# helixml/helix

Measured on AMD Instinct MI355X. Metric: tokens/sec, higher is better.
Workload: dtype bf16; 1 GPU; model=llama3-8b, global_batch=512, seq_len=512, parallelism=dp1, kv_cache_dtype=bf16

## Files before the change

### helix_amd/engine/engine.py

```python
from __future__ import annotations

import time
import zlib
from dataclasses import dataclass, field
from enum import Enum
from typing import Callable, Dict, List, Optional

import numpy as np
import torch

from helix_amd import ops
from helix_amd.engine.kv_cache import KVCache, chain_hash
from helix_amd.engine.sampling_params import SamplingParams
from helix_amd.models.llama import (DecodeMeta, LlamaConfig, LlamaForCausalLM,
                                    PrefillMeta, PRESETS)

_SEED_MIX = 0x9E3779B97F4A7C15


class SeqStatus(Enum):
    WAITING = "waiting"
    RUNNING = "running"
    FINISHED = "finished"
    CANCELLED = "cancelled"


@dataclass
class Sequence:
    seq_id: str
    prompt_ids: List[int]
    params: SamplingParams
    output_ids: List[int] = field(default_factory=list)
    status: SeqStatus = SeqStatus.WAITING
    block_table: List[int] = field(default_factory=list)
    row: int = -1
    cached_prefix: int = 0
    block_hashes: List[bytes] = field(default_factory=list)
    arrival_time: float = field(default_factory=time.monotonic)
    first_token_time: Optional[float] = None
    finish_reason: Optional[str] = None
    logprobs: List[dict] = field(default_factory=list)
    pen_init: bool = False
    json_mask: object = None
    on_token: Optional[Callable] = None
    lora: Optional[str] = None

    @property
    def total_len(self) -> int:
        return len(self.prompt_ids) + len(self.output_ids)


@dataclass
class EngineConfig:
    model: str = "llama3-8b"
    block_size: int = 16
    max_num_seqs: int = 64
    max_model_len: int = 8192
    max_prefill_tokens: int = 8192
    kv_cache_blocks: Optional[int] = None
    gpu_memory_utilization: float = 0.90
    eos_token_id: int = 2
    seed: int = 0
    enforce_eager: bool = False
    enable_prefix_caching: bool = True
    quantization: Optional[str] = None
    kv_cache_dtype: str = "bf16"
    max_loras: int = 0
    max_lora_rank: int = 16


class LLMEngine:
    def __init__(self, cfg: EngineConfig, device: str = "cuda",
                 model: Optional[LlamaForCausalLM] = None,
                 tp_size: int = 1, tp_rank: int = 0,
                 tp_group=None):
        self.cfg = cfg
        self.device = torch.device(device)
        self.model_cfg: LlamaConfig = PRESETS[cfg.model]
        self.tp_size = tp_size
        self.tp_rank = tp_rank
        self.tp_group = tp_group
        if model is None:
            dtype = torch.bfloat16
            model = LlamaForCausalLM(self.model_cfg, tp_size, tp_rank)
            model = model.to(dtype).to(self.device)
            model.init_random(cfg.seed)
        if cfg.quantization == "fp8":
            from helix_amd.models.quant import quantize_model_fp8
            quantize_model_fp8(model)
        elif cfg.quantization in ("q4_0", "q8_0", "q4_k", "q6_k"):
            from helix_amd.models.quant import has_wq, quantize_model_wq
            if not has_wq(model):
                quantize_model_wq(model, cfg.quantization)
        from helix_amd.models.quant import attach_wq_scratch
        attach_wq_scratch(model)
        self.model = model
        self.lora = None
        if cfg.max_loras > 0:
            if tp_size > 1:
                raise ValueError(
                    "max_loras > 0 is not supported with tp_size > 1 "
                    "(tensor-parallel-sharded adapters are not implemented)")
            from helix_amd.models.lora import LoRAManager
            self.lora = LoRAManager(model, cfg.max_loras, cfg.max_lora_rank)

        nkv = self.model_cfg.num_kv_heads // tp_size
        num_blocks = cfg.kv_cache_blocks
        if num_blocks is None:
            num_blocks = self._auto_kv_blocks(nkv)
        kv_dtype = torch.uint8 if cfg.kv_cache_dtype == "fp8" \
            else torch.bfloat16
        self.kv = KVCache(self.model_cfg.num_layers, nkv,
                          self.model_cfg.head_dim, cfg.block_size, num_blocks,
                          self.device, dtype=kv_dtype)
        self.waiting: List[Sequence] = []
        self.running: List[Sequence] = []
        self.seqs: Dict[str, Sequence] = {}
        self.steps = 0
        if self.device.type == "cuda":
            self.decode_ws = ops.decode_workspace(
                cfg.max_num_seqs, self.model_cfg.num_heads // tp_size,
                self.model_cfg.head_dim, cfg.max_model_len, self.device)
        else:
            self.decode_ws = None
        self._pen_counts: Optional[torch.Tensor] = None
        self._pen_seen: Optional[torch.Tensor] = None
        if self.device.type == "cuda":
            R = cfg.max_num_seqs
            self._samp_hf = torch.empty(5, R, dtype=torch.float32,
                                        pin_memory=True)
            self._samp_hs = torch.empty(R, dtype=torch.int64,
                                        pin_memory=True)
            self._samp_hi = torch.empty(2, R, dtype=torch.int32,
                                        pin_memory=True)
            self._samp_df = torch.empty(5, R, dtype=torch.float32,
                                        device=self.device)
            self._samp_ds = torch.empty(R, dtype=torch.int64,
                                        device=self.device)
            self._samp_di = torch.empty(2, R, dtype=torch.int32,
                                        device=self.device)
        mb = cfg.max_model_len // cfg.block_size + 2
        self._bt_np = np.zeros((cfg.max_num_seqs, mb), dtype=np.int32)
        self._free_rows = list(range(cfg.max_num_seqs - 1, -1, -1))
        self._ids_np = np.zeros(cfg.max_num_seqs, dtype=np.int64)
        self._pos_np = np.zeros(cfg.max_num_seqs, dtype=np.int64)
        self._slots_np = np.zeros(cfg.max_num_seqs, dtype=np.int64)
        self._lens_np = np.zeros(cfg.max_num_seqs, dtype=np.int32)
        self._rows_np = np.zeros(cfg.max_num_seqs, dtype=np.intp)
        self._lora_np = np.full(cfg.max_num_seqs, -1, dtype=np.int32)
        self.graph_runner = None
        if self.device.type == "cuda" and not cfg.enforce_eager:
            from helix_amd.engine.graph_runner import CUDAGraphRunner
            self.graph_runner = CUDAGraphRunner(
                self.model, self.kv.caches, self.decode_ws,
                cfg.max_model_len, cfg.block_size, cfg.max_num_seqs,
                self.device, lora=self.lora is not None)

    def _auto_kv_blocks(self, nkv: int) -> int:
        if self.device.type != "cuda":
            return 512
        free, total = torch.cuda.mem_get_info(self.device)
        budget = int(total * self.cfg.gpu_memory_utilization
                     - (total - free))
        budget = max(budget, 1 << 28)
        n = KVCache.blocks_for_bytes(budget, self.model_cfg.num_layers, nkv,
                                     self.model_cfg.head_dim,
                                     self.cfg.block_size)
        cap = (self.cfg.max_num_seqs *
               (self.cfg.max_model_len // self.cfg.block_size + 1))
        return max(1, min(n, cap))

    def add_request(self, seq_id: str, prompt_ids: List[int],
                    params: SamplingParams,
                    on_token: Optional[Callable] = None,
                    lora: Optional[str] = None) -> Sequence:
        if len(prompt_ids) >= self.cfg.max_model_len:
            raise ValueError(
                f"prompt length {len(prompt_ids)} >= max_model_len "
                f"{self.cfg.max_model_len}")
        if lora is not None:
            if self.lora is None:
                raise ValueError(
                    f"LoRA adapter {lora!r} requested but the engine was "
                    "built with max_loras=0")
            if lora not in self.lora.adapters:
                raise ValueError(f"unknown LoRA adapter {lora!r}")
        seq = Sequence(seq_id=seq_id, prompt_ids=list(prompt_ids),
                       params=params, on_token=on_token, lora=lora)
        self.seqs[seq_id] = seq
        self.waiting.append(seq)
        return seq

    def _lora_in_use(self, name: str) -> bool:
        return any(s.lora == name for s in self.waiting + self.running)

    def add_lora(self, name: str, path: str):
        if self.lora is None:
            raise ValueError("engine was built with max_loras=0")
        if self._lora_in_use(name):
            raise ValueError(
                f"LoRA adapter {name!r} is referenced by queued or running "
                "sequences; cannot reload it")
        self.lora.add(name, path)

    def remove_lora(self, name: str):
        if self.lora is None or name not in self.lora.adapters:
            raise ValueError(f"unknown LoRA adapter {name!r}")
        if self._lora_in_use(name):
            raise ValueError(
                f"LoRA adapter {name!r} is referenced by queued or running "
                "sequences; cannot remove it")
        self.lora.remove(name)

    def list_loras(self) -> List[str]:
        return self.lora.names() if self.lora is not None else []

    def _pinned_loras(self, batch: List[Sequence]) -> set:
        pinned = {s.lora for s in self.running if s.lora}
        pinned.update(s.lora for s in batch if s.lora)
        pinned.update(s.lora for s in self.waiting
                      if s.lora and s.block_table)
        return pinned

    def _lora_slots(self, lora_names) -> Optional[List[int]]:
        if self.lora is None or not any(lora_names):
            return None
        out = []
        for n in lora_names:
            s = self.lora.slot_of(n)
            if n is not None and s < 0:
                raise RuntimeError(f"LoRA adapter {n!r} is not resident")
            out.append(s)
        return out

    def cancel(self, seq_id: str):
        seq = self.seqs.get(seq_id)
        if seq is None:
            return
        if seq.status == SeqStatus.WAITING:
            self.waiting.remove(seq)
            if seq.block_table:
                self.kv.allocator.free(seq.block_table)
                seq.block_table = []
                self._release_row(seq)
        elif seq.status == SeqStatus.RUNNING:
            self.running.remove(seq)
            self.kv.allocator.free(seq.block_table)
            seq.block_table = []
            self._release_row(seq)
        seq.status = SeqStatus.CANCELLED
        seq.finish_reason = "cancelled"

    @property
    def has_work(self) -> bool:
        return bool(self.waiting or self.running)

    def num_free_blocks(self) -> int:
        return self.kv.allocator.free_count

    def step(self) -> List[tuple]:
        prefill_batch = self._schedule_prefill()
        if prefill_batch:
            out = self._run_prefill(prefill_batch)
        elif self.running:
            out = self._run_decode()
        else:
            return []
        self.steps += 1
        events = []
        for seq, tok in out:
            finished = self._append_token(seq, tok)
            events.append((seq, tok, finished))
            if seq.on_token is not None:
                seq.on_token(seq, tok, finished)
        return events

    def _schedule_prefill(self) -> List[Sequence]:
        batch: List[Sequence] = []
        tokens = 0
        bs = self.cfg.block_size
        alloc = self.kv.allocator
        self._chunk_target: Dict[str, int] = {}
        while self.waiting and len(self.running) + len(batch) < self.cfg.max_num_seqs:
            seq = self.waiting[0]
            L = len(seq.prompt_ids)
            first = not seq.block_table
            if seq.lora is not None and self.lora.acquire(
                    seq.lora, self._pinned_loras(batch)) < 0:
                break
            matched: List[int] = []
            if first:
                if self.cfg.enable_prefix_caching:
                    if not seq.block_hashes:
                        h = b"" if seq.lora is None \
                            else self.lora.hash_seed(seq.lora)
                        for i in range(L // bs):
                            h = chain_hash(h,
                                           seq.prompt_ids[i * bs:(i + 1) * bs])
                            seq.block_hashes.append(h)
                    for h in seq.block_hashes:
                        b = alloc.lookup_hash(h)
                        if b is None:
                            break
                        matched.append(b)
                    while matched and len(matched) * bs > L - 1:
                        matched.pop()
                P = len(matched) * bs
            else:
                P = seq.cached_prefix
            budget = self.cfg.max_prefill_tokens - tokens
            if budget <= 0:
                break
            T = min(L, P + budget)
            if T <= P:
                break
            if batch and T < L:
                break
            nblocks = (T + bs - 1) // bs
            new_blocks = nblocks - max(len(seq.block_table), len(matched))
            head = 1 if T == L else 0
            if not alloc.can_allocate(new_blocks + head):
                break
            if first:
                seq.block_table = [alloc.share(b) for b in matched] + \
                    alloc.allocate(new_blocks)
            else:
                seq.block_table.extend(alloc.allocate(new_blocks))
            self._assign_row(seq)
            seq.cached_prefix = P
            self._chunk_target[seq.seq_id] = T
            if T == L:
                batch.append(self.waiting.pop(0))
            else:
                batch.append(seq)
            tokens += T - P
            if T < L:
                break
        return batch

    def _slot(self, seq: Sequence, pos: int) -> int:
        bs = self.cfg.block_size
        return seq.block_table[pos // bs] * bs + pos % bs

    def _assign_row(self, seq: Sequence):
        if seq.row < 0:
            seq.row = self._free_rows.pop()
        n = len(seq.block_table)
        self._bt_np[seq.row, :n] = seq.block_table
        self._bt_np[seq.row, n:] = 0

    def _release_row(self, seq: Sequence):
        if seq.row >= 0:
            self._free_rows.append(seq.row)
            seq.row = -1
        seq.pen_init = False

    def _run_prefill(self, batch: List[Sequence]):
        bs = self.cfg.block_size
        input_ids, positions, slots, cu_q, cu_k = [], [], [], [0], [0]
        gather_blk, gather_off = [], []
        row_slots = self._lora_slots([s.lora for s in batch])
        tok_slots: List[int] = []
        targets = getattr(self, "_chunk_target", {})
        any_cached = any(s.cached_prefix for s in batch)
        for seq in batch:
            L = targets.get(seq.seq_id, len(seq.prompt_ids))
            P = seq.cached_prefix
            input_ids.extend(seq.prompt_ids[P:L])
            positions.extend(range(P, L))
            slots.extend(self._slot(seq, p) for p in range(P, L))
            cu_q.append(cu_q[-1] + L - P)
            cu_k.append(cu_k[-1] + L)
            if row_slots is not None:
                tok_slots.extend([row_slots[len(cu_q) - 2]] * (L - P))
            if any_cached:
                for p in range(L):
                    gather_blk.append(seq.block_table[p // bs])
                    gather_off.append(p % bs)
        dev = self.device
        meta = PrefillMeta(
            cu_seqlens=torch.tensor(cu_q, dtype=torch.int32, device=dev),
            max_seqlen=max(targets.get(s.seq_id, len(s.prompt_ids))
                           - s.cached_prefix for s in batch),
            slot_mapping=torch.tensor(slots, dtype=torch.int64, device=dev),
            positions=torch.tensor(positions, dtype=torch.int64, device=dev),
            cu_seqlens_k=(torch.tensor(cu_k, dtype=torch.int32, device=dev)
                          if any_cached else None),
            gather_blk=(torch.tensor(gather_blk, dtype=torch.int64,
                                     device=dev) if any_cached else None),
            gather_off=(torch.tensor(gather_off, dtype=torch.int64,
                                     device=dev) if any_cached else None),
            lora_slots=(torch.tensor(tok_slots, dtype=torch.int32,
                                     device=dev)
                        if row_slots is not None else None))
        ids = torch.tensor(input_ids, dtype=torch.int64, device=dev)
        hidden = self.model(ids, self.kv.caches, meta)
        if self.cfg.enable_prefix_caching:
            for seq in batch:
                T = targets.get(seq.seq_id, len(seq.prompt_ids))
                start = seq.cached_prefix // bs
                end = min(len(seq.block_hashes), T // bs)
                for i in range(start, end):
                    self.kv.allocator.register_hash(seq.block_table[i],
                                                    seq.block_hashes[i])
        last_rows = torch.tensor([c - 1 for c in cu_q[1:]], dtype=torch.int64,
                                 device=dev)
        logits = self.model.compute_logits(hidden[last_rows])
        tokens = self._sample(batch, logits)
        now = time.monotonic()
        out = []
        for seq, tok in zip(batch, tokens):
            T = targets.get(seq.seq_id, len(seq.prompt_ids))
            if T < len(seq.prompt_ids):
                seq.cached_prefix = T
                continue
            seq.status = SeqStatus.RUNNING
            seq.first_token_time = now
            self.running.append(seq)
            out.append((seq, tok))
        return out

    def _preempt_for_blocks(self):
        for w in self.waiting:
            if w.block_table:
                self.kv.allocator.free(w.block_table)
                w.block_table = []
                w.cached_prefix = 0
                self._release_row(w)
                return w
        if len(self.running) <= 1:
            return None
        victim = self.running.pop()
        self.kv.allocator.free(victim.block_table)
        victim.block_table = []
        self._release_row(victim)
        victim.prompt_ids = victim.prompt_ids + victim.output_ids
        victim.output_ids = []
        victim.cached_prefix = 0
        victim.block_hashes = []
        victim.status = SeqStatus.WAITING
        self.waiting.insert(0, victim)
        return victim

    def _run_decode(self):
        bs = self.cfg.block_size
        dev = self.device
        batch = []
        preempted = set()
        nb_ = 0
        ids_np, pos_np = self._ids_np, self._pos_np
        slots_np, lens_np, rows_np = self._slots_np, self._lens_np, self._rows_np
        for seq in list(self.running):
            if seq.seq_id in preempted:
                continue
            pos = seq.total_len - 1
            nblk = pos // bs + 1
            while len(seq.block_table) < nblk:
                if not self.kv.allocator.can_allocate(1):
                    victim = self._preempt_for_blocks()
                    if victim is None:
                        raise RuntimeError(
                            "KV cache exhausted and nothing to preempt")
                    preempted.add(victim.seq_id)
                    if victim is seq:
                        break
                    continue
                seq.block_table.extend(self.kv.allocator.allocate(1))
                self._bt_np[seq.row, len(seq.block_table) - 1] = \
                    seq.block_table[-1]
            if seq.seq_id in preempted:
                continue
            batch.append(seq)
            ids_np[nb_] = (seq.output_ids[-1] if seq.output_ids
                           else seq.prompt_ids[-1])
            pos_np[nb_] = pos
            slots_np[nb_] = self._slot(seq, pos)
            lens_np[nb_] = pos + 1
            rows_np[nb_] = seq.row
            if self.lora is not None:
                ls = self.lora.slot_of(seq.lora)
                if ls < 0 and seq.lora is not None:
                    raise RuntimeError(
                        f"LoRA adapter {seq.lora!r} is not resident")
                self._lora_np[nb_] = ls
            nb_ += 1
        if not batch:
            return []
        B = nb_
        max_blocks = max(len(s.block_table) for s in batch)
        bt_np = self._bt_np[rows_np[:B], :max_blocks]
        max_len = int(lens_np[:B].max())
        if self.graph_runner is not None:
            logits = self.graph_runner.run(ids_np[:B], pos_np[:B],
                                           slots_np[:B], bt_np,
                                           lens_np[:B], max_len,
                                           lora_slots=(self._lora_np[:B]
                                                       if self.lora is not None
                                                       else None))
        else:
            row_slots = self._lora_slots([s.lora for s in batch])
            meta = DecodeMeta(
                block_tables=torch.from_numpy(bt_np).to(dev),
                seq_lens=torch.from_numpy(lens_np[:B].copy()).to(dev),
                slot_mapping=torch.from_numpy(slots_np[:B].copy()).to(dev),
                positions=torch.from_numpy(pos_np[:B].copy()).to(dev),
                max_len=max_len,
                workspace=self.decode_ws,
                lora_slots=(torch.tensor(row_slots, dtype=torch.int32,
                                         device=dev)
                            if row_slots is not None else None))
            ids = torch.from_numpy(ids_np[:B].copy()).to(dev)
            hidden = self.model(ids, self.kv.caches, meta)
            logits = self.model.compute_logits(hidden)
        tokens = self._sample(batch, logits)
        return list(zip(batch, tokens))

    def _ensure_pen_row(self, seq: Sequence):
        if self._pen_counts is None:
            V = self.model_cfg.vocab_size
            R = self.cfg.max_num_seqs
            self._pen_counts = torch.zeros(R, V, dtype=torch.int32,
                                           device=self.device)
            self._pen_seen = torch.zeros(R, V, dtype=torch.uint8,
                                         device=self.device)
        if not seq.pen_init and seq.row >= 0:
            row = seq.row
            self._pen_counts[row].zero_()
            self._pen_seen[row].zero_()
            pid = torch.tensor(seq.prompt_ids, dtype=torch.int64,
                               device=self.device)
            self._pen_seen[row][pid] = 1
            if seq.output_ids:
                oid = torch.tensor(seq.output_ids, dtype=torch.int64,
                                   device=self.device)
                self._pen_counts[row].index_put_(
                    (oid,), torch.ones(len(seq.output_ids),
                                       dtype=torch.int32,
                                       device=self.device),
                    accumulate=True)
            seq.pen_init = True

    def _apply_json_masks(self, batch: List[Sequence],
                          logits: torch.Tensor):
        from helix_amd.engine.json_mode import JSONByteMask
        from helix_amd.utils.tokenizer import N_SPECIAL
        for i, s in enumerate(batch):
            if not s.params.json_mode:
                continue
            if s.json_mask is None:
                s.json_mask = JSONByteMask()
            m = s.json_mask
            if m.complete:
                allowed = [self.cfg.eos_token_id]                     if self.cfg.eos_token_id >= 0 else []
            else:
                V = logits.shape[1]
                allowed = [b + N_SPECIAL for b in m.allowed_bytes()
                           if b + N_SPECIAL < V]
            row = logits[i]
            if not allowed:
                continue
            idx = torch.tensor(allowed, dtype=torch.int64,
                               device=row.device)
            keep = row[idx].clone()
            row.fill_(float("-inf"))
            row[idx] = keep

    def _advance_json_masks(self, batch: List[Sequence],
                            out: List[int]):
        from helix_amd.utils.tokenizer import N_SPECIAL
        for i, s in enumerate(batch):
            if s.params.json_mode and s.json_mask is not None:
                b = out[i] - N_SPECIAL
                if 0 <= b < 256:
                    s.json_mask.push_byte(b)

    def _sample(self, batch: List[Sequence], logits: torch.Tensor) -> List[int]:
        B = len(batch)
        needs_bias = any(s.params.logit_bias for s in batch)
        needs_json = any(s.params.json_mode for s in batch)
        if needs_bias or needs_json:
            logits = logits.clone()
        if needs_bias:
            for i, s in enumerate(batch):
                lb = s.params.logit_bias
                if not lb:
                    continue
                idx = torch.tensor([int(k) for k in lb],
                                   dtype=torch.int64,
                                   device=logits.device)
                vals = torch.tensor([float(v) for v in lb.values()],
                                    dtype=logits.dtype,
                                    device=logits.device)
                logits[i].index_add_(0, idx, vals)
        if needs_json:
            self._apply_json_masks(batch, logits)
        lp_rows = [i for i, s_ in enumerate(batch) if s_.params.logprobs]
        needs_proc = any(s.params.needs_logit_processing for s in batch)
        gpu_fast = logits.is_cuda and needs_proc
        if needs_proc and not gpu_fast:
            logits = self._process_logits(
                batch, logits.float().clone()
                if logits.is_inference() else logits.float())
        elif gpu_fast and lp_rows:
            sub = logits[lp_rows].float().clone()
            self._process_logits([batch[i] for i in lp_rows], sub)
            if logits.is_inference():
                logits = logits.clone()
            logits[lp_rows] = sub.to(logits.dtype)
        on_gpu = logits.is_cuda
        if on_gpu:
            hf = self._samp_hf.numpy()
            hs = self._samp_hs.numpy()
        else:
            hf = np.empty((5, B), dtype=np.float32)
            hs = np.empty(B, dtype=np.int64)
        sig = (tuple(s.seq_id for s in batch), tuple(lp_rows),
               gpu_fast, on_gpu)
        cache = getattr(self, "_samp_cache", None)
        if cache is not None and cache["sig"] == sig:
            cache["outlens"] += 1
            hs[:B] = (cache["base"] + cache["outlens"] * _SEED_MIX)                 & 0x7FFFFFFFFFFFFFFF
            hf[0, :B] = cache["temps"]
        else:
            base_v = np.empty(B, dtype=np.uint64)
            outlen_v = np.empty(B, dtype=np.uint64)
            for i, s in enumerate(batch):
                hf[0, i] = s.params.temperature
                base_v[i] = s.params.seed if s.params.seed is not None                     else (zlib.crc32(s.seq_id.encode()) & 0x7FFFFFFF)
                outlen_v[i] = len(s.output_ids)
            hs[:B] = (base_v + outlen_v * _SEED_MIX)                 & 0x7FFFFFFFFFFFFFFF
            self._samp_cache = {"sig": sig, "base": base_v,
                                "outlens": outlen_v,
                                "temps": hf[0, :B].copy(),
                                "params_done": False}
            cache = self._samp_cache
        if gpu_fast:
            hi = self._samp_hi.numpy()
            if cache.get("params_done"):
                pen_idx = cache["pen_idx"]
                hf[1:5, :B] = cache["pf"]
                hi[:, :B] = cache["pi"]
            else:
                lp_set = set(lp_rows)
                hf[1, :B] = 1.0
                hf[2, :B] = 1.0
                hf[3, :B] = 0.0
                hf[4, :B] = 0.0
                hi[0, :B] = 0
                hi[1, :B] = -1
                pen_idx = []
                for i, s in enumerate(batch):
                    if i in lp_set:
                        continue
                    p = s.params
                    hf[1, i] = p.top_p
                    hi[0, i] = p.top_k
                    if (p.repetition_penalty != 1.0
                            or p.presence_penalty != 0.0
                            or p.frequency_penalty != 0.0):
                        hf[2, i] = p.repetition_penalty
                        hf[3, i] = p.presence_penalty
                        hf[4, i] = p.frequency_penalty
                        self._ensure_pen_row(s)
                        hi[1, i] = s.row
                        pen_idx.append(i)
                cache["pen_idx"] = pen_idx
                cache["pf"] = hf[1:5, :B].copy()
                cache["pi"] = hi[:, :B].copy()
                cache["params_done"] = True
            dev = logits.device
            self._samp_df[:, :B].copy_(self._samp_hf[:, :B],
                                       non_blocking=True)
            self._samp_ds[:B].copy_(self._samp_hs[:B], non_blocking=True)
            self._samp_di[:, :B].copy_(self._samp_hi[:, :B],
                                       non_blocking=True)
            toks = ops.sample_tokens_ext(
                logits.contiguous(), self._samp_df[0, :B],
                self._samp_ds[:B], self._samp_df[1, :B],
                self._samp_di[0, :B], self._samp_df[2, :B],
                self._samp_df[3, :B], self._samp_df[4, :B],
                self._pen_counts, self._pen_seen, self._samp_di[1, :B])
            if pen_idx:
                rows_t = torch.tensor([batch[i].row for i in pen_idx],
                                      dtype=torch.int64, device=dev)
                sel = toks[pen_idx]
                self._pen_counts.index_put_(
                    (rows_t, sel), torch.ones(len(pen_idx),
                                              dtype=torch.int32, device=dev),
                    accumulate=True)
        elif on_gpu:
            self._samp_df[0, :B].copy_(self._samp_hf[0, :B],
                                       non_blocking=True)
            self._samp_ds[:B].copy_(self._samp_hs[:B], non_blocking=True)
            toks = ops.sample_tokens(logits.contiguous(),
                                     self._samp_df[0, :B],
                                     self._samp_ds[:B])
        else:
            temps = torch.from_numpy(hf[0, :B].copy())
            seeds_t = torch.from_numpy(hs[:B].copy())
            toks = ops.sample_tokens(logits.contiguous(), temps, seeds_t)
        out = toks.cpu().tolist()
        if any(s.params.json_mode for s in batch):
            self._advance_json_masks(batch, out)
        lp_rows = [i for i, s_ in enumerate(batch) if s_.params.logprobs]
        if lp_rows:
            k = max(batch[i].params.logprobs for i in lp_rows)
            sub = logits[lp_rows].float()
            lsm = torch.log_softmax(sub, dim=-1)
            topv, topi = lsm.topk(min(k, lsm.shape[-1]), dim=-1)
            topv = topv.cpu().tolist()
            topi = topi.cpu().tolist()
            for j, i in enumerate(lp_rows):
                tok = out[i]
                tok_lp = float(lsm[j, tok])
                kk = batch[i].params.logprobs
                batch[i].logprobs.append({
                    "token": tok, "logprob": tok_lp,
                    "top_logprobs": [
                        {"token": t, "logprob": v}
                        for t, v in zip(topi[j][:kk], topv[j][:kk])]})
        return out

    def _process_logits(self, batch, logits: torch.Tensor) -> torch.Tensor:
        for i, seq in enumerate(batch):
            p = seq.params
            if p.repetition_penalty != 1.0 or p.presence_penalty != 0.0 \
               or p.frequency_penalty != 0.0:
                seen = torch.tensor(
                    list(set(seq.prompt_ids + seq.output_ids)),
                    dtype=torch.int64, device=logits.device)
                row = logits[i]
                if p.repetition_penalty != 1.0:
                    vals = row[seen]
                    row[seen] = torch.where(vals > 0,
                                            vals / p.repetition_penalty,
                                            vals * p.repetition_penalty)
                if p.presence_penalty != 0.0:
                    row[seen] -= p.presence_penalty
                if p.frequency_penalty != 0.0:
                    from collections import Counter
                    cnt = Counter(seq.output_ids)
                    idx = torch.tensor(list(cnt.keys()), dtype=torch.int64,
                                       device=logits.device)
                    freq = torch.tensor(list(cnt.values()),
                                        dtype=torch.float32,
                                        device=logits.device)
                    row[idx] -= p.frequency_penalty * freq
            if p.top_k > 0:
                kth = torch.topk(logits[i], p.top_k).values[-1]
                logits[i][logits[i] < kth] = -float("inf")
            if p.top_p < 1.0:
                sorted_logits, idx = torch.sort(logits[i], descending=True)
                probs = torch.softmax(sorted_logits, -1)
                cum = probs.cumsum(-1)
                cut = (cum - probs) >= p.top_p
                sorted_logits[cut] = -float("inf")
                logits[i].scatter_(0, idx, sorted_logits)
        return logits

    def _append_token(self, seq: Sequence, tok: int) -> bool:
        seq.output_ids.append(tok)
        p = seq.params
        finished = None
        if not p.ignore_eos and (tok == self.cfg.eos_token_id
                                 or tok in p.stop_token_ids):
            finished = "stop"
        elif len(seq.output_ids) >= p.max_tokens:
            finished = "length"
        elif seq.total_len >= self.cfg.max_model_len:
            finished = "length"
        if finished:
            seq.status = SeqStatus.FINISHED
            seq.finish_reason = finished
            self.running.remove(seq)
            self.kv.allocator.free(seq.block_table)
            seq.block_table = []
            self._release_row(seq)
            return True
        return False

    def generate(self, prompts: List[List[int]],
                 params: SamplingParams,
                 loras: Optional[List[Optional[str]]] = None
                 ) -> List[List[int]]:
        self._gen_calls = getattr(self, "_gen_calls", 0) + 1
        ids = [f"gen-{self._gen_calls}-{i}"
               for i in range(len(prompts))]
        if loras is None:
            loras = [None] * len(prompts)
        if len(loras) != len(prompts):
            raise ValueError("loras must have one entry per prompt")
        for sid, p, lo in zip(ids, prompts, loras):
            self.add_request(sid, p, params, lora=lo)
        while self.has_work:
            self.step()
        return [self.seqs[sid].output_ids for sid in ids]
```

### helix_amd/engine/kv_cache.py

```python
from __future__ import annotations

import hashlib
from typing import Dict, List, Optional, Tuple

import torch


def chain_hash(prev: bytes, tokens: List[int]) -> bytes:
    h = hashlib.blake2b(digest_size=16)
    h.update(prev)
    h.update(b"|")
    h.update(",".join(map(str, tokens)).encode())
    return h.digest()


class BlockAllocator:

    def __init__(self, num_blocks: int):
        self.num_blocks = num_blocks
        self._free: List[int] = list(range(num_blocks - 1, -1, -1))
        from collections import OrderedDict
        self._cached_free: "OrderedDict[int, None]" = OrderedDict()
        self.ref: Dict[int, int] = {}
        self._hash_to_block: Dict[bytes, int] = {}
        self._block_hash: Dict[int, bytes] = {}

    @property
    def free_count(self) -> int:
        return len(self._free) + len(self._cached_free)

    def can_allocate(self, n: int) -> bool:
        return self.free_count >= n

    def _drop_hash(self, b: int):
        h = self._block_hash.pop(b, None)
        if h is not None and self._hash_to_block.get(h) == b:
            self._hash_to_block.pop(h, None)

    def allocate(self, n: int) -> List[int]:
        if n > self.free_count:
            raise RuntimeError(
                f"KV cache exhausted: need {n} blocks, "
                f"{self.free_count} free")
        out: List[int] = []
        for _ in range(n):
            if self._free:
                b = self._free.pop()
            else:
                b, _ = self._cached_free.popitem(last=False)
                self._drop_hash(b)
            self.ref[b] = 1
            out.append(b)
        return out

    def share(self, block: int) -> int:
        if block in self._cached_free:
            del self._cached_free[block]
        self.ref[block] = self.ref.get(block, 0) + 1
        return block

    def free(self, blocks: List[int]):
        for b in blocks:
            r = self.ref.get(b, 1) - 1
            if r <= 0:
                self.ref.pop(b, None)
                if b in self._block_hash:
                    self._cached_free[b] = None
                else:
                    self._free.append(b)
            else:
                self.ref[b] = r

    def register_hash(self, block: int, h: bytes):
        old = self._hash_to_block.get(h)
        if old is not None and old != block and old in self._cached_free:
            del self._cached_free[old]
            self._block_hash.pop(old, None)
            self._free.append(old)
        self._hash_to_block[h] = block
        self._block_hash[block] = h

    def lookup_hash(self, h: bytes) -> Optional[int]:
        b = self._hash_to_block.get(h)
        if b is None:
            return None
        if self.ref.get(b, 0) > 0 or b in self._cached_free:
            return b
        return None


class KVCache:

    def __init__(self, num_layers: int, num_kv_heads: int, head_dim: int,
                 block_size: int, num_blocks: int, device, dtype=torch.bfloat16):
        self.block_size = block_size
        self.num_blocks = num_blocks
        self.caches = []
        for _ in range(num_layers):
            k = torch.zeros(num_blocks, num_kv_heads, block_size, head_dim,
                            dtype=dtype, device=device)
            v = torch.zeros(num_blocks, num_kv_heads, block_size, head_dim,
                            dtype=dtype, device=device)
            self.caches.append((k, v))
        self.allocator = BlockAllocator(num_blocks)

    @staticmethod
    def block_bytes(num_layers: int, num_kv_heads: int, head_dim: int,
                    block_size: int, dtype=torch.bfloat16) -> int:
        el = torch.empty(0, dtype=dtype).element_size()
        return 2 * num_layers * num_kv_heads * block_size * head_dim * el

    @staticmethod
    def blocks_for_bytes(budget: int, num_layers: int, num_kv_heads: int,
                         head_dim: int, block_size: int) -> int:
        return max(0, budget // KVCache.block_bytes(
            num_layers, num_kv_heads, head_dim, block_size))
```

### helix_amd/ops/hip/paged_attn_decode.hip

```cpp
#include "common.h"
#include <torch/extension.h>
#include <ATen/hip/HIPContext.h>

using namespace helix;

namespace {

constexpr int NTHREADS = 128;
constexpr int CHUNK = 128;
constexpr int MAX_G = 8;
constexpr int PART_QUANT = 128;
constexpr int MAX_PARTS = 512;
constexpr int TARGET_WGS = 1024;

template <bool KV8> struct CacheElem;
template <> struct CacheElem<false> {
  using elem = uint16_t;
  using kvec = u16x8;
  using vvec = u16x8;
  static constexpr int KVEC = 8;
  static __device__ __forceinline__ float to_f32(uint16_t x) {
    return bf16_to_f32(x);
  }
};
template <> struct CacheElem<true> {
  using elem = uint8_t;
  using kvec = u8x16;
  using vvec = u8x8;
  static constexpr int KVEC = 16;
  static __device__ __forceinline__ float to_f32(uint8_t x) {
    return fp8_to_f32(x);
  }
};

template <int DHEAD, int G, bool KV8, int VPS>
__global__ __launch_bounds__(NTHREADS, 2) void paged_attn_decode_kernel(
    uint16_t* __restrict__ out,
    float* __restrict__ tmp_out,
    float* __restrict__ tmp_ml,
    const uint16_t* __restrict__ q,
    const uint16_t* __restrict__ k_cache,
    const uint16_t* __restrict__ v_cache,
    const int* __restrict__ block_tables,
    const int* __restrict__ seq_lens,
    float scale, int Hkv, int block_size, int max_blocks,
    int partition_size, int max_parts, int window) {
  using CE = CacheElem<KV8>;
  using elem_t = typename CE::elem;
  using kvec_t = typename CE::kvec;
  using vvec_t = typename CE::vvec;
  constexpr int KVEC = CE::KVEC;

  const int seq = blockIdx.x;
  const int hkv = blockIdx.y;
  const int part = blockIdx.z;
  const int nparts = gridDim.z;
  const int Hq = Hkv * G;
  const int len = seq_lens[seq];
  const int kv_lo = (window > 0) ? max(0, len - window) : 0;
  int p_start = part * partition_size;
  const int p_hi = min(len, p_start + partition_size);
  if (p_start < kv_lo) p_start = kv_lo;
  if (p_start >= len || p_hi <= kv_lo) {
    if (nparts > 1 && threadIdx.x == 0) {
#pragma unroll
      for (int g = 0; g < G; ++g) {
        const int hq = hkv * G + g;
        float* ml = tmp_ml + (((int64_t)seq * Hq + hq) * max_parts + part) * 2;
        ml[0] = -INFINITY;
        ml[1] = 0.f;
      }
    }
    return;
  }
  const int p_end = p_hi;

  __shared__ float q_lds[G][DHEAD];
  __shared__ float s_lds[G][CHUNK];
  __shared__ float head_m[MAX_G], head_l[MAX_G], head_corr[MAX_G];

  for (int idx = threadIdx.x; idx < G * DHEAD; idx += NTHREADS) {
    const int g = idx / DHEAD, d = idx % DHEAD;
    q_lds[g][d] =
        bf16_to_f32(q[((int64_t)seq * Hq + hkv * G + g) * DHEAD + d]) * scale;
  }
  if (threadIdx.x < MAX_G) {
    head_m[threadIdx.x] = -INFINITY;
    head_l[threadIdx.x] = 0.f;
  }
  __syncthreads();

  constexpr int NGRP = DHEAD / 8;
  constexpr int C_PAR = NTHREADS / NGRP;
  const int d8 = (threadIdx.x % NGRP) * 8;
  const int cpar = threadIdx.x / NGRP;
  float acc[G][8];
#pragma unroll
  for (int g = 0; g < G; ++g)
#pragma unroll
    for (int i = 0; i < 8; ++i) acc[g][i] = 0.f;

  const int* btable = block_tables + (int64_t)seq * max_blocks;
  const int nwaves = NTHREADS / WAVE;
  const int wid = threadIdx.x / WAVE;
  const int lane = threadIdx.x & (WAVE - 1);

  kvec_t kpre[DHEAD / KVEC];
  auto issue_kpre = [&](int cbase) {
    const int tok = min(cbase + (int)threadIdx.x, p_end - 1);
    const int64_t roff =
        (((int64_t)btable[tok / block_size] * Hkv + hkv) *
             (int64_t)block_size + tok % block_size) * DHEAD;
    const elem_t* krow = (const elem_t*)k_cache + roff;
#pragma unroll
    for (int j = 0; j < DHEAD / KVEC; ++j)
      kpre[j] = *reinterpret_cast<const kvec_t*>(krow + j * KVEC);
  };
  issue_kpre(p_start);

  for (int base = p_start; base < p_end; base += CHUNK) {
    const int chunk_n = min(CHUNK, p_end - base);

    if ((int)threadIdx.x < chunk_n) {
      float s[G];
#pragma unroll
      for (int g = 0; g < G; ++g) s[g] = 0.f;
#pragma unroll
      for (int j = 0; j < DHEAD / KVEC; ++j) {
        float kv[KVEC];
#pragma unroll
        for (int i = 0; i < KVEC; ++i) kv[i] = CE::to_f32(kpre[j][i]);
#pragma unroll
        for (int g = 0; g < G; ++g) {
#pragma unroll
          for (int i = 0; i < KVEC; ++i)
            s[g] += q_lds[g][j * KVEC + i] * kv[i];
        }
      }
#pragma unroll
      for (int g = 0; g < G; ++g) s_lds[g][threadIdx.x] = s[g];
    }
    if (base + CHUNK < p_end) issue_kpre(base + CHUNK);
    __syncthreads();

    for (int g = wid; g < G; g += nwaves) {
      float m_chunk = -INFINITY;
      for (int i = lane; i < chunk_n; i += WAVE)
        m_chunk = fmaxf(m_chunk, s_lds[g][i]);
      m_chunk = wave_reduce_max(m_chunk);
      const float m_old = head_m[g];
      const float m_new = fmaxf(m_old, m_chunk);
      const float corr = (m_old == -INFINITY) ? 0.f : __expf(m_old - m_new);
      float l_add = 0.f;
      for (int i = lane; i < chunk_n; i += WAVE) {
        const float p = __expf(s_lds[g][i] - m_new);
        s_lds[g][i] = p;
        l_add += p;
      }
      l_add = wave_reduce_sum(l_add);
      if (lane == 0) {
        head_l[g] = head_l[g] * corr + l_add;
        head_m[g] = m_new;
        head_corr[g] = corr;
      }
    }
    __syncthreads();

    {
#pragma unroll
      for (int g = 0; g < G; ++g)
#pragma unroll
        for (int i = 0; i < 8; ++i) acc[g][i] *= head_corr[g];
      const int npass = (chunk_n - cpar + C_PAR - 1) / C_PAR;
      auto vrow_off = [&](int tok) {
        const int64_t blk = btable[tok / block_size];
        return (((blk * Hkv + hkv) * (int64_t)block_size +
                 tok % block_size)) * DHEAD + d8;
      };
      auto load_v = [&](int64_t off, float v[8]) {
        const vvec_t raw =
            *reinterpret_cast<const vvec_t*>((const elem_t*)v_cache + off);
#pragma unroll
        for (int i = 0; i < 8; ++i) v[i] = CE::to_f32(raw[i]);
      };
      int ps = 0;
      if constexpr (!KV8) {
        for (; ps + VPS <= npass; ps += VPS) {
          u16x8 vraw[VPS];
#pragma unroll
          for (int u = 0; u < VPS; ++u)
            vraw[u] = *reinterpret_cast<const u16x8*>(
                v_cache + vrow_off(base + (ps + u) * C_PAR + cpar));
#pragma unroll
          for (int u = 0; u < VPS; ++u) {
            const int tok_i = (ps + u) * C_PAR + cpar;
            float v[8];
#pragma unroll
            for (int i = 0; i < 8; ++i) v[i] = bf16_to_f32(vraw[u][i]);
#pragma unroll
            for (int g = 0; g < G; ++g) {
              const float pv = s_lds[g][tok_i];
#pragma unroll
              for (int i = 0; i < 8; ++i) acc[g][i] += pv * v[i];
            }
          }
        }
      } else {
        for (; ps + VPS <= npass; ps += VPS) {
          int64_t voff[VPS];
#pragma unroll
          for (int u = 0; u < VPS; ++u)
            voff[u] = vrow_off(base + (ps + u) * C_PAR + cpar);
          float v4[VPS][8];
#pragma unroll
          for (int u = 0; u < VPS; ++u) load_v(voff[u], v4[u]);
#pragma unroll
          for (int u = 0; u < VPS; ++u) {
            const int tok_i = (ps + u) * C_PAR + cpar;
#pragma unroll
            for (int g = 0; g < G; ++g) {
              const float pv = s_lds[g][tok_i];
#pragma unroll
              for (int i = 0; i < 8; ++i) acc[g][i] += pv * v4[u][i];
            }
          }
        }
      }
      for (; ps < npass; ++ps) {
        const int tok_i = ps * C_PAR + cpar;
        float v[8];
        load_v(vrow_off(base + tok_i), v);
#pragma unroll
        for (int g = 0; g < G; ++g) {
          const float pv = s_lds[g][tok_i];
#pragma unroll
          for (int i = 0; i < 8; ++i) acc[g][i] += pv * v[i];
        }
      }
    }
    __syncthreads();
  }

  __shared__ float comb[G * DHEAD];
#pragma unroll
  for (int g = 0; g < G; ++g) {
    if (cpar == 0) {
#pragma unroll
      for (int i = 0; i < 8; ++i) comb[g * DHEAD + d8 + i] = acc[g][i];
    }
  }
  __syncthreads();
  for (int p = 1; p < C_PAR; ++p) {
    if (cpar == p) {
#pragma unroll
      for (int g = 0; g < G; ++g)
#pragma unroll
        for (int i = 0; i < 8; ++i)
          comb[g * DHEAD + d8 + i] += acc[g][i];
    }
    __syncthreads();
  }
  if (cpar == 0) {
#pragma unroll
    for (int g = 0; g < G; ++g) {
      const int hq = hkv * G + g;
      if (nparts == 1) {
        const float inv_l = 1.f / fmaxf(head_l[g], 1e-20f);
        float o[8];
#pragma unroll
        for (int i = 0; i < 8; ++i)
          o[i] = comb[g * DHEAD + d8 + i] * inv_l;
        store_bf16x8(out + ((int64_t)seq * Hq + hq) * DHEAD + d8, o);
      } else {
        float* tp =
            tmp_out + (((int64_t)seq * Hq + hq) * max_parts + part) * DHEAD;
#pragma unroll
        for (int i = 0; i < 8; ++i) tp[d8 + i] = comb[g * DHEAD + d8 + i];
        if (d8 == 0) {
          float* ml =
              tmp_ml + (((int64_t)seq * Hq + hq) * max_parts + part) * 2;
          ml[0] = head_m[g];
          ml[1] = head_l[g];
        }
      }
    }
  }
}

__global__ __launch_bounds__(128) void paged_attn_reduce_kernel(
    uint16_t* __restrict__ out, const float* __restrict__ tmp_out,
    const float* __restrict__ tmp_ml, const int* __restrict__ seq_lens,
    int Hq, int D, int partition_size, int max_parts) {
  const int seq = blockIdx.x;
  const int hq = blockIdx.y;
  const int nparts =
      min(max_parts, (seq_lens[seq] + partition_size - 1) / partition_size);
  const float* ml = tmp_ml + ((int64_t)seq * Hq + hq) * max_parts * 2;

  __shared__ float w[MAX_PARTS];
  __shared__ float l_sh;
  if (threadIdx.x == 0) {
    float M = -INFINITY;
    for (int p = 0; p < nparts; ++p) M = fmaxf(M, ml[p * 2]);
    float L = 0.f;
    for (int p = 0; p < nparts; ++p) {
      const float e = (ml[p * 2] == -INFINITY) ? 0.f : __expf(ml[p * 2] - M);
      w[p] = e;
      L += e * ml[p * 2 + 1];
    }
    l_sh = fmaxf(L, 1e-20f);
  }
  __syncthreads();
  const float* tp = tmp_out + ((int64_t)seq * Hq + hq) * max_parts * D;
  for (int d = threadIdx.x; d < D; d += blockDim.x) {
    float o = 0.f;
    for (int p = 0; p < nparts; ++p) {
      if (w[p] != 0.f) o += w[p] * tp[p * D + d];
    }
    out[((int64_t)seq * Hq + hq) * D + d] = f32_to_bf16(o / l_sh);
  }
}

template <int DHEAD, int G>
void launch_decode(uint16_t* out, float* tmp_out, float* tmp_ml,
                   const uint16_t* q, const uint16_t* kc, const uint16_t* vc,
                   const int* bt, const int* lens, float scale, int B,
                   int Hkv, int block_size, int max_blocks, int eff_part,
                   int nparts, int max_parts, int window, bool kv8,
                   hipStream_t stream) {
#define LAUNCH_PD(K8, VPS)                                                   \
  hipLaunchKernelGGL((paged_attn_decode_kernel<DHEAD, G, K8, VPS>),          \
                     dim3(B, Hkv, nparts), dim3(NTHREADS), 0, stream, out,   \
                     tmp_out, tmp_ml, q, kc, vc, bt, lens, scale, Hkv,       \
                     block_size, max_blocks, eff_part, max_parts, window)
  if (kv8)                          LAUNCH_PD(true, 4);
  else if (B * Hkv * nparts < 2048) LAUNCH_PD(false, 8);
  else                              LAUNCH_PD(false, 4);
#undef LAUNCH_PD
}

}

int64_t decode_part_quant() { return PART_QUANT; }

void paged_attn_decode(torch::Tensor out, torch::Tensor q,
                       torch::Tensor k_cache, torch::Tensor v_cache,
                       torch::Tensor block_tables, torch::Tensor seq_lens,
                       double scale, torch::Tensor tmp_out,
                       torch::Tensor tmp_ml, int64_t max_len,
                       int64_t window) {
  const int B = q.size(0);
  const int Hq = q.size(1);
  const int D = q.size(2);
  const int Hkv = k_cache.size(1);
  const int block_size = k_cache.size(2);
  const int max_blocks = block_tables.size(1);
  const int max_parts = tmp_out.dim() == 4 ? tmp_out.size(2) : 0;
  TORCH_CHECK(D == 64 || D == 128, "head_dim must be 64 or 128");
  TORCH_CHECK(Hkv > 0 && Hq % Hkv == 0, "Hq must be a multiple of Hkv");
  const int G = Hq / Hkv;
  TORCH_CHECK(G == 1 || G == 2 || G == 4 || G == 8, "G must be 1/2/4/8");
  TORCH_CHECK(max_len >= 1, "max_len must be >= 1, got ", max_len);
  TORCH_CHECK(q.scalar_type() == torch::kBFloat16 &&
                  out.scalar_type() == torch::kBFloat16,
              "q and out must be bf16");
  TORCH_CHECK(k_cache.scalar_type() == v_cache.scalar_type(),
              "k_cache and v_cache must share a dtype");
  TORCH_CHECK(block_tables.scalar_type() == torch::kInt32,
              "block_tables must be int32");
  TORCH_CHECK(seq_lens.scalar_type() == torch::kInt32,
              "seq_lens must be int32");
  TORCH_CHECK(seq_lens.size(0) == B && block_tables.size(0) == B,
              "seq_lens and block_tables must have B = ", B, " rows");
  TORCH_CHECK(q.is_contiguous() && out.is_contiguous() &&
                  k_cache.is_contiguous() && v_cache.is_contiguous() &&
                  block_tables.is_contiguous() && seq_lens.is_contiguous() &&
                  tmp_out.is_contiguous() && tmp_ml.is_contiguous(),
              "paged_attn_decode takes contiguous tensors");
  TORCH_CHECK(tmp_out.scalar_type() == torch::kFloat32 && max_parts >= 1 &&
                  tmp_out.sizes() == at::IntArrayRef({B, Hq, max_parts, D}),
              "tmp_out must be fp32 [B, Hq, max_parts, D] with B = ", B,
              ", Hq = ", Hq, ", D = ", D, "; got ", tmp_out.sizes());
  TORCH_CHECK(tmp_ml.scalar_type() == torch::kFloat32 &&
                  tmp_ml.sizes() == at::IntArrayRef({B, Hq, max_parts, 2}),
              "tmp_ml must be fp32 [B, Hq, max_parts, 2] with tmp_out's "
              "max_parts = ", max_parts, "; got ", tmp_ml.sizes());

  const int max_useful = cdiv((int)max_len, PART_QUANT);
  int nparts = std::max(1, TARGET_WGS / std::max(1, B * Hkv));
  nparts = std::min({nparts, max_useful, max_parts, MAX_PARTS});
  int eff_part = cdiv(cdiv((int)max_len, nparts), PART_QUANT) * PART_QUANT;
  nparts = cdiv((int)max_len, eff_part);

  auto stream = at::hip::getCurrentHIPStream();
  auto* o = (uint16_t*)out.data_ptr();
  auto* to = tmp_out.data_ptr<float>();
  auto* tm = tmp_ml.data_ptr<float>();
  auto* qp = (const uint16_t*)q.data_ptr();
  auto* kp = (const uint16_t*)k_cache.data_ptr();
  auto* vp = (const uint16_t*)v_cache.data_ptr();
  auto* bp = block_tables.data_ptr<int>();
  auto* lp = seq_lens.data_ptr<int>();

  const bool kv8 = k_cache.scalar_type() == torch::kUInt8;
#define DISPATCH(DH, GG)                                                     \
  launch_decode<DH, GG>(o, to, tm, qp, kp, vp, bp, lp, (float)scale, B,     \
                        Hkv, block_size, max_blocks, eff_part, nparts,      \
                        max_parts, (int)window, kv8, stream)
  if (D == 128) {
    if (G == 1) DISPATCH(128, 1);
    else if (G == 2) DISPATCH(128, 2);
    else if (G == 4) DISPATCH(128, 4);
    else DISPATCH(128, 8);
  } else {
    if (G == 1) DISPATCH(64, 1);
    else if (G == 2) DISPATCH(64, 2);
    else if (G == 4) DISPATCH(64, 4);
    else DISPATCH(64, 8);
  }
#undef DISPATCH

  if (nparts > 1) {
    hipLaunchKernelGGL(paged_attn_reduce_kernel, dim3(B, Hq), dim3(128), 0,
                       stream, o, to, tm, lp, Hq, D, eff_part, max_parts);
  }
}
```

Measured before the change: 26840 tokens/s.

## Stage block-table ids in LDS and use power-of-two block indexing in decode

```diff
diff --git a/helix_amd/engine/engine.py b/helix_amd/engine/engine.py
--- a/helix_amd/engine/engine.py
+++ b/helix_amd/engine/engine.py
@@ -10,7 +10,7 @@
 import torch
 
 from helix_amd import ops
-from helix_amd.engine.kv_cache import KVCache, chain_hash
+from helix_amd.engine.kv_cache import KVCache, chain_hash, check_block_size
 from helix_amd.engine.sampling_params import SamplingParams
 from helix_amd.models.llama import (DecodeMeta, LlamaConfig, LlamaForCausalLM,
                                     PrefillMeta, PRESETS)
@@ -67,6 +67,9 @@
     kv_cache_dtype: str = "bf16"
     max_loras: int = 0
     max_lora_rank: int = 16
+
+    def __post_init__(self):
+        check_block_size(self.block_size)
 
 
 class LLMEngine:
diff --git a/helix_amd/engine/kv_cache.py b/helix_amd/engine/kv_cache.py
--- a/helix_amd/engine/kv_cache.py
+++ b/helix_amd/engine/kv_cache.py
@@ -89,11 +89,22 @@
         return None
 
 
+MIN_BLOCK_SIZE = 8
+
+
+def check_block_size(block_size: int) -> int:
+    if block_size < MIN_BLOCK_SIZE or block_size & (block_size - 1):
+        raise ValueError(
+            f"block_size must be a power of two and at least "
+            f"{MIN_BLOCK_SIZE}, got {block_size}")
+    return block_size
+
+
 class KVCache:
 
     def __init__(self, num_layers: int, num_kv_heads: int, head_dim: int,
                  block_size: int, num_blocks: int, device, dtype=torch.bfloat16):
-        self.block_size = block_size
+        self.block_size = check_block_size(block_size)
         self.num_blocks = num_blocks
         self.caches = []
         for _ in range(num_layers):
diff --git a/helix_amd/ops/hip/paged_attn_decode.hip b/helix_amd/ops/hip/paged_attn_decode.hip
--- a/helix_amd/ops/hip/paged_attn_decode.hip
+++ b/helix_amd/ops/hip/paged_attn_decode.hip
@@ -1,4 +1,5 @@
 #include "common.h"
+#include <type_traits>
 #include <torch/extension.h>
 #include <ATen/hip/HIPContext.h>
 
@@ -12,6 +13,8 @@
 constexpr int PART_QUANT = 128;
 constexpr int MAX_PARTS = 512;
 constexpr int TARGET_WGS = 1024;
+constexpr int MIN_BS = 8;
+constexpr int IDS_MAX = CHUNK / MIN_BS + 1;
 
 template <bool KV8> struct CacheElem;
 template <> struct CacheElem<false> {
@@ -34,7 +37,9 @@
 };
 
 template <int DHEAD, int G, bool KV8, int VPS>
-__global__ __launch_bounds__(NTHREADS, 2) void paged_attn_decode_kernel(
+__global__ __launch_bounds__(NTHREADS,
+                             (G <= 2 && (DHEAD == 64 || KV8)) ? 4 : 2)
+void paged_attn_decode_kernel(
     uint16_t* __restrict__ out,
     float* __restrict__ tmp_out,
     float* __restrict__ tmp_ml,
@@ -43,7 +48,7 @@
     const uint16_t* __restrict__ v_cache,
     const int* __restrict__ block_tables,
     const int* __restrict__ seq_lens,
-    float scale, int Hkv, int block_size, int max_blocks,
+    float scale, int Hkv, int bs_log2, int max_blocks,
     int partition_size, int max_parts, int window) {
   using CE = CacheElem<KV8>;
   using elem_t = typename CE::elem;
@@ -78,11 +83,36 @@
   __shared__ float q_lds[G][DHEAD];
   __shared__ float s_lds[G][CHUNK];
   __shared__ float head_m[MAX_G], head_l[MAX_G], head_corr[MAX_G];
-
-  for (int idx = threadIdx.x; idx < G * DHEAD; idx += NTHREADS) {
-    const int g = idx / DHEAD, d = idx % DHEAD;
-    q_lds[g][d] =
-        bf16_to_f32(q[((int64_t)seq * Hq + hkv * G + g) * DHEAD + d]) * scale;
+  __shared__ int blk_ids[3][IDS_MAX];
+
+  const int* btable = block_tables + (int64_t)seq * max_blocks;
+  const int bs_mask = (1 << bs_log2) - 1;
+  auto load_id = [&](int cbase) {
+    const int last = (min(cbase + CHUNK, p_end) - 1) >> bs_log2;
+    return btable[min((cbase >> bs_log2) + (int)threadIdx.x, last)];
+  };
+  const int id0 = load_id(p_start);
+  const int id1 = load_id(min(p_start + CHUNK, p_end - 1));
+
+  {
+    constexpr int QV = G * DHEAD >= NTHREADS ? G * DHEAD / NTHREADS : 1;
+    typedef __attribute__((ext_vector_type(QV))) uint16_t qvec_t;
+    const int idx = threadIdx.x * QV;
+    if (idx < G * DHEAD) {
+      const uint16_t* qp = q + ((int64_t)seq * Hq + hkv * G) * DHEAD + idx;
+      float* dst = &q_lds[0][0] + idx;
+      if constexpr (QV == 1) {
+        dst[0] = bf16_to_f32(qp[0]) * scale;
+      } else {
+        const qvec_t raw = *reinterpret_cast<const qvec_t*>(qp);
+#pragma unroll
+        for (int i = 0; i < QV; ++i) dst[i] = bf16_to_f32(raw[i]) * scale;
+      }
+    }
+  }
+  if (threadIdx.x < IDS_MAX) {
+    blk_ids[0][threadIdx.x] = id0;
+    blk_ids[1][threadIdx.x] = id1;
   }
   if (threadIdx.x < MAX_G) {
     head_m[threadIdx.x] = -INFINITY;
@@ -94,34 +124,42 @@
   constexpr int C_PAR = NTHREADS / NGRP;
   const int d8 = (threadIdx.x % NGRP) * 8;
   const int cpar = threadIdx.x / NGRP;
+  if constexpr (G == 8 && !KV8) __builtin_assume(cpar < C_PAR);
   float acc[G][8];
 #pragma unroll
   for (int g = 0; g < G; ++g)
 #pragma unroll
     for (int i = 0; i < 8; ++i) acc[g][i] = 0.f;
 
-  const int* btable = block_tables + (int64_t)seq * max_blocks;
   const int nwaves = NTHREADS / WAVE;
   const int wid = threadIdx.x / WAVE;
   const int lane = threadIdx.x & (WAVE - 1);
 
+  auto row_off = [&](int buf, int cbase, int tok) {
+    const int64_t blk =
+        blk_ids[buf][(tok >> bs_log2) - (cbase >> bs_log2)];
+    return (((blk * Hkv + hkv) << bs_log2) + (tok & bs_mask)) * DHEAD;
+  };
+
   kvec_t kpre[DHEAD / KVEC];
-  auto issue_kpre = [&](int cbase) {
+  auto issue_kpre = [&](int buf, int cbase) {
     const int tok = min(cbase + (int)threadIdx.x, p_end - 1);
-    const int64_t roff =
-        (((int64_t)btable[tok / block_size] * Hkv + hkv) *
-             (int64_t)block_size + tok % block_size) * DHEAD;
-    const elem_t* krow = (const elem_t*)k_cache + roff;
+    const elem_t* krow = (const elem_t*)k_cache + row_off(buf, cbase, tok);
 #pragma unroll
     for (int j = 0; j < DHEAD / KVEC; ++j)
       kpre[j] = *reinterpret_cast<const kvec_t*>(krow + j * KVEC);
   };
-  issue_kpre(p_start);
-
-  for (int base = p_start; base < p_end; base += CHUNK) {
-    const int chunk_n = min(CHUNK, p_end - base);
-
-    if ((int)threadIdx.x < chunk_n) {
+  issue_kpre(0, p_start);
+
+  int cur = 0, nxt = 1, aft = 2;
+
+  auto do_chunk = [&](auto has_next, const int base) {
+    constexpr bool HAS_NEXT = decltype(has_next)::value;
+    const int chunk_n = HAS_NEXT ? CHUNK : p_end - base;
+    const int npass = (chunk_n - cpar + C_PAR - 1) / C_PAR;
+    auto vrow_off = [&](int tok) { return row_off(cur, base, tok) + d8; };
+
+    if (HAS_NEXT || (int)threadIdx.x < chunk_n) {
       float s[G];
 #pragma unroll
       for (int g = 0; g < G; ++g) s[g] = 0.f;
@@ -140,7 +178,11 @@
 #pragma unroll
       for (int g = 0; g < G; ++g) s_lds[g][threadIdx.x] = s[g];
     }
-    if (base + CHUNK < p_end) issue_kpre(base + CHUNK);
+    const bool stage_ids = HAS_NEXT && base + 2 * CHUNK < p_end;
+    int id_aft = 0;
+    if constexpr (HAS_NEXT)
+      id_aft = load_id(min(base + 2 * CHUNK, p_end - 1));
+    if constexpr (HAS_NEXT) issue_kpre(nxt, base + CHUNK);
     __syncthreads();
 
     for (int g = wid; g < G; g += nwaves) {
@@ -171,12 +213,8 @@
       for (int g = 0; g < G; ++g)
 #pragma unroll
         for (int i = 0; i < 8; ++i) acc[g][i] *= head_corr[g];
-      const int npass = (chunk_n - cpar + C_PAR - 1) / C_PAR;
-      auto vrow_off = [&](int tok) {
-        const int64_t blk = btable[tok / block_size];
-        return (((blk * Hkv + hkv) * (int64_t)block_size +
-                 tok % block_size)) * DHEAD + d8;
-      };
+      if (stage_ids && threadIdx.x < IDS_MAX)
+        blk_ids[aft][threadIdx.x] = id_aft;
       auto load_v = [&](int64_t off, float v[8]) {
         const vvec_t raw =
             *reinterpret_cast<const vvec_t*>((const elem_t*)v_cache + off);
@@ -239,7 +277,15 @@
       }
     }
     __syncthreads();
-  }
+    const int t = cur;
+    cur = nxt;
+    nxt = aft;
+    aft = t;
+  };
+  int base = p_start;
+  for (; base + CHUNK < p_end; base += CHUNK)
+    do_chunk(std::true_type{}, base);
+  do_chunk(std::false_type{}, base);
 
   __shared__ float comb[G * DHEAD];
 #pragma unroll
@@ -325,14 +371,14 @@
 void launch_decode(uint16_t* out, float* tmp_out, float* tmp_ml,
                    const uint16_t* q, const uint16_t* kc, const uint16_t* vc,
                    const int* bt, const int* lens, float scale, int B,
-                   int Hkv, int block_size, int max_blocks, int eff_part,
+                   int Hkv, int bs_log2, int max_blocks, int eff_part,
                    int nparts, int max_parts, int window, bool kv8,
                    hipStream_t stream) {
 #define LAUNCH_PD(K8, VPS)                                                   \
   hipLaunchKernelGGL((paged_attn_decode_kernel<DHEAD, G, K8, VPS>),          \
                      dim3(B, Hkv, nparts), dim3(NTHREADS), 0, stream, out,   \
                      tmp_out, tmp_ml, q, kc, vc, bt, lens, scale, Hkv,       \
-                     block_size, max_blocks, eff_part, max_parts, window)
+                     bs_log2, max_blocks, eff_part, max_parts, window)
   if (kv8)                          LAUNCH_PD(true, 4);
   else if (B * Hkv * nparts < 2048) LAUNCH_PD(false, 8);
   else                              LAUNCH_PD(false, 4);
@@ -361,6 +407,11 @@
   const int G = Hq / Hkv;
   TORCH_CHECK(G == 1 || G == 2 || G == 4 || G == 8, "G must be 1/2/4/8");
   TORCH_CHECK(max_len >= 1, "max_len must be >= 1, got ", max_len);
+  TORCH_CHECK(block_size >= MIN_BS && (block_size & (block_size - 1)) == 0,
+              "KV cache block_size must be a power of two and at least ",
+              MIN_BS, ", got ", block_size);
+  int bs_log2 = 0;
+  while ((1 << bs_log2) < block_size) ++bs_log2;
   TORCH_CHECK(q.scalar_type() == torch::kBFloat16 &&
                   out.scalar_type() == torch::kBFloat16,
               "q and out must be bf16");
@@ -377,6 +428,8 @@
                   block_tables.is_contiguous() && seq_lens.is_contiguous() &&
                   tmp_out.is_contiguous() && tmp_ml.is_contiguous(),
               "paged_attn_decode takes contiguous tensors");
+  TORCH_CHECK(reinterpret_cast<uintptr_t>(q.data_ptr()) % 16 == 0,
+              "q must be 16-byte aligned (it is read with vector loads)");
   TORCH_CHECK(tmp_out.scalar_type() == torch::kFloat32 && max_parts >= 1 &&
                   tmp_out.sizes() == at::IntArrayRef({B, Hq, max_parts, D}),
               "tmp_out must be fp32 [B, Hq, max_parts, D] with B = ", B,
@@ -405,7 +458,7 @@
   const bool kv8 = k_cache.scalar_type() == torch::kUInt8;
 #define DISPATCH(DH, GG)                                                     \
   launch_decode<DH, GG>(o, to, tm, qp, kp, vp, bp, lp, (float)scale, B,     \
-                        Hkv, block_size, max_blocks, eff_part, nparts,      \
+                        Hkv, bs_log2, max_blocks, eff_part, nparts,         \
                         max_parts, (int)window, kv8, stream)
   if (D == 128) {
     if (G == 1) DISPATCH(128, 1);
```

Result: faster. 28350 tokens/s, median of 6 (+5.6%).
